# pritishnahar95/nvidia-terraform-modules

Hardware: AMD Instinct MI355X
Metric: cluster time-to-GPU-ready (s) + validation HIP GEMM TFLOPS at 1/2/4/8 MI355X (higher is better)
Workload: dtype bf16

## Files before the change

### nvidia_terraform_modules_amd/ops/_lib.py

```python
from __future__ import annotations

import ctypes
import os
from pathlib import Path

import torch

_HERE = Path(__file__).resolve().parent
LIB_PATH = _HERE / "libntm_validation.so"
EXP_LIB_PATH = _HERE / "libntm_experimental.so"

_lib: ctypes.CDLL | None = None
_exp: ctypes.CDLL | None = None


class NativeLibraryMissing(RuntimeError):
    pass


c_int, c_size, c_float, c_vp = ctypes.c_int, ctypes.c_size_t, ctypes.c_float, ctypes.c_void_p
c_uint, c_u64, c_double = ctypes.c_uint, ctypes.c_ulonglong, ctypes.c_double
_c_vpp = ctypes.POINTER(c_vp)

SIGNATURES = {
# ... 94 lines not shown
    "ntm_cu_sweep_launch": ([c_vp, c_vp, c_uint, c_int, c_size, c_uint,
                             c_uint, c_int, c_vp], c_int),
    "ntm_cu_sweep_decode": ([c_uint, c_uint, c_vp], None),
    "ntm_cu_sweep_summarize": ([c_vp, c_size, c_uint, c_uint, c_int, c_vp, c_size],
                               c_size),
    "ntm_xcd_sweep_record_bytes": ([], c_int),
    "ntm_xcd_sweep_heads_bytes": ([], c_int),
    "ntm_xcd_sweep_tile_bytes": ([], c_int),
    "ntm_xcd_sweep_mfma_per_batch": ([], c_int),
    "ntm_xcd_sweep_gated": ([c_int, c_int], c_int),
    "ntm_xcd_sweep_read_launch": ([c_vp, c_size, c_uint, c_uint, c_uint, c_int,
                                   c_u64, c_uint, c_int, c_uint, c_vp, c_vp,
                                   c_vp], c_int),
    "ntm_xcd_sweep_mfma_launch": ([c_uint, c_uint, c_uint, c_uint,
                                   c_uint, c_int, c_uint, c_vp, c_vp, c_vp], c_int),
    "ntm_xcd_sweep_summarize": ([c_vp, c_size, c_int, c_int, c_uint, c_uint,
                                 c_u64, c_double, c_int, c_vp, c_size], c_size),
    "ntm_atomics_ops": ([], c_int),
    "ntm_atomics_op_name": ([c_int], ctypes.c_char_p),
    "ntm_atomics_slot_bytes": ([c_int], c_int),
    "ntm_atomics_record_bytes": ([], c_int),
    "ntm_atomics_exact": ([c_int, c_u64, c_u64], c_int),
    "ntm_atomics_rmw_shape_ok": ([c_int, c_u64, c_uint, c_uint, c_u64], c_int),
    "ntm_atomics_expected": ([c_int, c_u64, c_u64, c_u64, c_u64, c_vp], c_int),
    "ntm_atomics_rmw_launch": ([c_int, c_vp, c_u64, c_uint, c_uint, c_u64, c_u64, c_vp], c_int),
    "ntm_atomics_rmw_reference_launch": ([c_int, c_vp, c_u64, c_uint, c_uint, c_u64, c_u64, c_vp], c_int),
    "ntm_atomics_ticket_claim_bytes": ([c_uint, c_uint, c_uint], c_size),
    "ntm_atomics_counter_bytes": ([c_uint], c_size),
    "ntm_atomics_ticket_launch": ([c_vp, c_vp, c_uint, c_uint, c_uint, c_uint, c_vp], c_int),
    "ntm_atomics_handoff_slab_bytes": ([c_uint, c_uint], c_size),
    "ntm_atomics_handoff_init": ([c_vp, c_uint, c_uint, c_u64, c_uint, c_vp], c_int),
    "ntm_atomics_handoff_launch": ([c_vp, c_vp, c_vp, c_uint, c_uint, c_u64, c_uint, c_uint, c_vp], c_int),
    "ntm_atomics_summarize_rmw": ([c_int, c_vp, c_vp, c_u64, c_int, c_vp, c_size], c_size),
    "ntm_atomics_summarize_tickets": ([c_vp, c_vp, c_uint, c_uint, c_uint, c_int, c_vp, c_size], c_size),
    "ntm_atomics_summarize_handoff": ([c_vp, c_size, c_uint, c_uint, c_uint, c_uint, c_int, c_vp, c_size], c_size),
}

XGMI_SIGNATURES = {
    "ntm_xgmi_allreduce_bf16": ([_c_vpp, _c_vpp, _c_vpp, c_int, c_int, c_int, c_int, c_size,
                                 c_uint, c_vp, c_int, c_vp], c_int),
    "ntm_xgmi_allreduce_bf16_ex": ([_c_vpp, _c_vpp, _c_vpp, c_int, c_int, c_int, c_int, c_size,
                                    c_uint, c_vp, c_int, c_uint, c_uint, c_vp], c_int),
    "ntm_xgmi_signal_bytes": ([c_int], c_size),
    "ntm_malloc": ([_c_vpp, c_size, c_int], c_int),
    "ntm_free": ([c_vp], c_int),
    "ntm_memset_async": ([c_vp, c_int, c_size, c_vp], c_int),
    "ntm_ipc_handle": ([c_vp, c_vp], c_int),
    "ntm_ipc_open": ([c_vp, _c_vpp], c_int),
    "ntm_ipc_close": ([c_vp], c_int),
}


def declare(lib: ctypes.CDLL, signatures: dict) -> None:
    for name, (argt, rest) in signatures.items():
        fn = getattr(lib, name)
        fn.argtypes = argt
        fn.restype = rest


def _declare(lib: ctypes.CDLL) -> None:
    declare(lib, SIGNATURES)


def lib() -> ctypes.CDLL:
    global _lib
    if _lib is not None:
        return _lib
    if not LIB_PATH.exists():
        raise NativeLibraryMissing(
            f"{LIB_PATH} not found. Build it with "
            "`python -m nvidia_terraform_modules_amd.ops.build` (needs hipcc, gfx950)."
        )
    mode = os.RTLD_NOW | getattr(os, "RTLD_GLOBAL", 0)
    _lib = ctypes.CDLL(str(LIB_PATH), mode=mode)
    _declare(_lib)
    return _lib


def _declare_experimental(lib: ctypes.CDLL) -> None:
    gemm = [c_int, c_vp, c_vp, c_vp, c_int, c_int, c_int, c_int, c_int, c_int, c_vp]
    sig = {
        "ntm_experimental_version": ([], ctypes.c_char_p),
        "ntm_gemm_bf16_experimental": (gemm, c_int),
        "ntm_gemm_bf16_knob": (gemm, c_int),
        "ntm_gemm_bf16_ws_knob": ([c_int] + gemm, c_int),
        "ntm_gemm_bf16_stamp": (
            [c_int, c_vp, c_vp, c_vp, c_int, c_int, c_int, c_int, c_int, c_int, c_vp, c_vp], c_int),
        "ntm_mfma_f8_probe": ([c_vp, c_vp, c_vp, c_vp], c_int),
        "ntm_mx_mfma_probe": ([c_int, c_vp, c_vp, c_vp, c_vp, c_vp, c_vp], c_int),
        "ntm_mfma_rate": ([c_int, c_int, c_int, c_vp, c_vp, c_vp], c_int),
        "ntm_mfma_toggle": ([c_int, c_int, c_int, c_vp, c_vp, c_vp], c_int),
        "ntm_dma_probe": ([c_int, c_vp, c_int, c_int, c_int, c_int, c_vp], c_int),
        "ntm_gemm_fp8_knob": ([c_vp, c_vp, c_vp, c_int, c_int, c_int, c_int, c_int, c_int, c_int,
                               c_vp], c_int),
        "ntm_gemm_bf16_sk_rev": ([c_vp, c_vp, c_vp, c_int, c_int, c_int, c_int, c_int, c_int,
                                  c_vp, c_size, c_vp], c_int),
        "ntm_gemm_bf16_sk_nopair": ([c_vp, c_vp, c_vp, c_int, c_int, c_int, c_int, c_int, c_int,
                                     c_vp, c_size, c_vp], c_int),
        "ntm_gemm_bf16_sk_stamp": ([c_vp, c_vp, c_vp, c_int, c_int, c_int, c_int, c_int, c_int,
                                    c_vp, c_size, c_vp, c_vp], c_int),
        "ntm_gemm_bf16_pp6_stamp": ([c_int, c_int, c_vp, c_vp, c_vp, c_int, c_int, c_int, c_int,
                                     c_int, c_int, c_vp, c_vp], c_int),
    }
    declare(lib, sig)


def lib_experimental() -> ctypes.CDLL:
    global _exp
    if _exp is not None:
        return _exp
    lib()
    if not EXP_LIB_PATH.exists():
        raise NativeLibraryMissing(
            f"{EXP_LIB_PATH} not found. Build it with "
            "`python -m nvidia_terraform_modules_amd.ops.build`.")
    _exp = ctypes.CDLL(str(EXP_LIB_PATH), mode=os.RTLD_NOW | getattr(os, "RTLD_GLOBAL", 0))
    _declare_experimental(_exp)
    return _exp


def available() -> bool:
    try:
        lib()
        return True
    except (NativeLibraryMissing, OSError):
        return False


def check(rc: int, what: str) -> None:
    if rc != 0:
        raise RuntimeError(f"{what} failed with hipError {rc}")


def stream_handle(stream: "torch.cuda.Stream | None" = None) -> int:
    if stream is None:
        stream = torch.cuda.current_stream()
    return int(stream.cuda_stream)


def version() -> str:
    return lib().ntm_version().decode()
```

### nvidia_terraform_modules_amd/ops/kernels.py

```python
from __future__ import annotations

import ctypes
from dataclasses import dataclass

import torch

from ._lib import check, lib, lib_experimental, stream_handle
from .mx import MX_BLOCK, mx_bits, mx_format_id, mx_shape_ok

BM = BN = 256
BK = 64


def gemm_shape_ok(m: int, n: int, k: int) -> bool:
    return m > 0 and n > 0 and k >= 2 * BK and m % BM == 0 and n % BN == 0 and k % BK == 0


def _require(t: torch.Tensor, name: str, dtype: torch.dtype) -> None:
    if not t.is_cuda:
        raise ValueError(f"{name} must be a GPU tensor")
    if t.dtype != dtype:
        raise ValueError(f"{name} must be {dtype}, got {t.dtype}")
    if t.dim() != 2 or t.stride(1) != 1:
        raise ValueError(f"{name} must be 2-D with unit inner stride")


GEMM_VARIANTS = {"default": 0, "pingpong8": 1, "pingpong8b": 4,
                 "pingpong8c": 5, "pingpong8cw": 10, "pingpong8cwe": 11,
                 "pingpong8cwn": 12, "pingpong8cwne": 13, "tile128": 15,
                 "tile256x128": 16, "tile160": 17, "tile256x160": 18, "tile128w4": 19,
                 "tile256x128w4": 20, "tile160w4": 21, "pingpong8cm": 22, "tile160x128": 23,
                 "tile128x160": 24, "tile128x256": 26, "pingpong8o": 25,
                 "pp8o_g128": 41, "pp8o_g128_nostore": 42, "pp8o_nostore": 43,
                 "pingpong8om": 47, "pingpong8od": 48, "pingpong8s": 49,
                 "pingpong8omd": 51, "pp192x256": 27, "pp256x192": 28,
                 "pp224x256": 29, "pp192x256s": 54, "pp256x192s": 55,
                 "dma4k_d3": 39}


EXPERIMENTAL_VARIANTS = frozenset({"pingpong8", "pingpong8cw",
                                   "pingpong8cwe", "pingpong8cwn", "pingpong8cwne",
                                   "tile128w4", "tile256x128w4", "tile160w4",
                                   "pp8o_g128", "pp8o_g128_nostore", "pp8o_nostore",
                                   "pingpong8od", "pingpong8omd", "pingpong8om", "pp224x256"})

TILE_SHAPES = {"tile128": (128, 128), "tile256x128": (256, 128), "tile160": (160, 160),
               "tile256x160": (256, 160), "tile128w4": (128, 128), "tile256x128w4": (256, 128),
               "tile160w4": (160, 160), "tile160x128": (160, 128), "tile128x160": (128, 160),
               "tile128x256": (128, 256)}


MASKED_TILES = frozenset({"tile128", "tile256x128", "tile160", "tile160x128", "tile128x160",
                          "tile128x256"})


def _tile128_shape_ok(m: int, n: int, k: int, tm: int = 128, tn: int = 128,
                      masked: bool = False) -> bool:
    if masked:
        return m > 0 and n > 0 and n % 4 == 0 and k > 0 and k % 8 == 0
    return m > 0 and n > 0 and m % tm == 0 and n % tn == 0 and k >= 128 and k % 128 == 0


def k1_plan(m: int, n: int, k: int) -> tuple[int, str, str]:
    top, tv, rest = ctypes.c_int(), ctypes.c_int(), ctypes.c_int()
    rc = lib().ntm_k1_plan(m, n, k, ctypes.byref(top), ctypes.byref(tv), ctypes.byref(rest))
    if rc != 0:
        raise ValueError(f"shape ({m},{n},{k}) not tiled by the K1 kernels")
    names = {v: kname for kname, v in GEMM_VARIANTS.items()}
    return top.value, names[tv.value], names[rest.value]


def k1_splitk_plan(m: int, n: int, k: int) -> tuple[int, str, str, int]:
    top, tv, rest, sp = ctypes.c_int(), ctypes.c_int(), ctypes.c_int(), ctypes.c_int()
    rc = lib().ntm_k1_plan_splitk(m, n, k, ctypes.byref(top), ctypes.byref(tv),
                                  ctypes.byref(rest), ctypes.byref(sp))
    if rc != 0:
        raise ValueError(f"shape ({m},{n},{k}) not tiled by the K1 kernels")
    names = {v: kname for kname, v in GEMM_VARIANTS.items()}
    return top.value, names[tv.value], names[rest.value], sp.value


_DEFAULT_WS: dict[tuple[int, int, int], int] = {}


_DEFAULT_SK: dict[tuple[int, int, int], str] = {}

SKH_VARIANTS = ("pp192x256s", "pp256x192s")
SK_VARIANTS = ("pingpong8s",) + SKH_VARIANTS


def k1_candidates(m: int, n: int, k: int, lda: int | None = None, ldb: int | None = None,
                  ldc: int | None = None) -> list[str]:
    lda, ldb, ldc = lda or k, ldb or k, ldc or n
    ok = (m % 256 == 0 and n % 256 == 0 and k % 128 == 0 and k >= 256 and
          not (lda % 8 or ldb % 8 or ldc % 8) and m * lda * 2 < (1 << 31) and
          n * ldb * 2 < (1 << 31))
    return ["default", "dma4k_d3"] if ok else ["default"]


def set_plan_pp_tiles(on: bool = True, split: bool | None = None) -> None:
    split = on if split is None else split
    lib().ntm_set_plan_pp_tiles((1 if on else 0) | (2 if split else 0))
    _DEFAULT_WS.clear()
    _DEFAULT_SK.clear()
    _FP8_WS.clear()


def set_plan_splitk(margin: float = 0.0, long_slice_k: int = -1, fp8: bool = True) -> None:
    lib().ntm_set_plan_splitk(float(margin), int(long_slice_k), 1 if fp8 else 0)
    _DEFAULT_WS.clear()
    _DEFAULT_SK.clear()
    _FP8_WS.clear()


def set_plan_splitk_ragged(on: bool = True) -> None:
    lib().ntm_set_plan_splitk_ragged(1 if on else 0)
    _DEFAULT_WS.clear()
    _DEFAULT_SK.clear()
    _FP8_WS.clear()


def set_cus_override(cus: int = 0) -> None:
    lib().ntm_set_cus_override(int(cus))
    _DEFAULT_WS.clear()
    _DEFAULT_SK.clear()
    _FP8_WS.clear()


def skh_ws_bytes(variant: str, m: int, n: int, k: int) -> int:
    if m <= 0 or n <= 0 or k <= 0:
        return 0
    return int(lib().ntm_skh_ws_bytes(GEMM_VARIANTS[variant], m, n, k))


def _default_ws_bytes(m: int, n: int, k: int) -> int:
    key = (m, n, k)
    wsb = _DEFAULT_WS.get(key)
    if wsb is None:
        _, top, _, sp = k1_splitk_plan(m, n, k)
        if top in SK_VARIANTS:
            ok = (sk_ws_bytes(m, n, k) if top == "pingpong8s" else skh_ws_bytes(top, m, n, k)) > 0
            wsb = -1 if ok else 0
            if ok:
                _DEFAULT_SK[key] = top
        else:
            wsb = lib().ntm_splitk_ws_bytes(m, n, k, sp) if sp > 1 else 0
        _DEFAULT_WS[key] = wsb
    return wsb


def gemm_bf16(a: torch.Tensor, b: torch.Tensor, out: torch.Tensor | None = None,
              variant: str = "default", splits: int = 1) -> torch.Tensor:
    _require(a, "a", torch.bfloat16)
    _require(b, "b", torch.bfloat16)
    m, k = a.shape
    n, kb = b.shape
    if k != kb:
        raise ValueError(f"K mismatch: a has {k}, b has {kb}")
    if variant in TILE_SHAPES:
        tm, tn = TILE_SHAPES[variant]
        if not _tile128_shape_ok(m, n, k, tm, tn, masked=variant in MASKED_TILES):
            raise ValueError(f"shape ({m},{n},{k}) not served by the {tm}x{tn} kernel "
                             "(masked tiles: N % 4, K % 8; others: whole tiles, K % 128)")
    elif variant == "default":
        _default_ws_bytes(m, n, k)
    elif variant in SKH_VARIANTS:
        if not skh_ws_bytes(variant, m, n, k):
            raise ValueError(f"shape ({m},{n},{k}) not served by {variant} (N % 8, K % 8, "
                             "K >= 128; at most half a round of its tiles, >= 2 K slices each)")
    elif variant in ("pingpong8s", "pingpong8s_rev", "pingpong8s_nopair"):
        if not sk_ws_bytes(m, n, k):
            raise ValueError(f"shape ({m},{n},{k}) not served by stream-K (N % 8, K % 8, K >= 128; "
                             "256x256 tiles: more than the CUs and not a multiple of them, or "
                             "few enough for >= 2 K slices per tile in one round)")
    elif variant in ("pingpong8cm", "pingpong8om", "pingpong8omd", "pp192x256", "pp256x192",
                     "pp224x256"):
        if not (m > 0 and n > 0 and n % 8 == 0 and k > 0 and k % 8 == 0):
            raise ValueError(f"shape ({m},{n},{k}) not served by {variant} (N % 8, K % 8)")
    elif not gemm_shape_ok(m, n, k):
        raise ValueError(f"shape ({m},{n},{k}) not tiled by the 256x256x64 kernel")
    if out is None:
        out = torch.empty((m, n), dtype=torch.bfloat16, device=a.device)
    _require(out, "out", torch.bfloat16)
    if tuple(out.shape) != (m, n):
        raise ValueError("out has the wrong shape")
    if variant in ("pingpong8s", "pingpong8s_rev", "pingpong8s_nopair"):
        return _gemm_bf16_sk(a, b, out, rev=variant == "pingpong8s_rev",
                             nopair=variant == "pingpong8s_nopair")
    if variant in SKH_VARIANTS:
        return _gemm_bf16_sk(a, b, out, sk_variant=variant)
    if splits > 1:
        if variant not in MASKED_TILES:
            raise ValueError(f"split-K runs on {sorted(MASKED_TILES)}, not {variant}")
        ws_bytes = lib().ntm_splitk_ws_bytes(m, n, k, splits)
        ws = torch.empty((ws_bytes + 3) // 4, dtype=torch.float32, device=a.device)
        rc = lib().ntm_gemm_bf16_splitk(
            GEMM_VARIANTS[variant], splits, a.data_ptr(), b.data_ptr(), out.data_ptr(), m, n, k,
            a.stride(0), b.stride(0), out.stride(0), ws.data_ptr(), ws_bytes, stream_handle())
        check(rc, "ntm_gemm_bf16_splitk")
        return out
    if variant.startswith("knob"):
        rc = lib_experimental().ntm_gemm_bf16_knob(
            int(variant[4:]), a.data_ptr(), b.data_ptr(), out.data_ptr(), m, n, k, a.stride(0),
            b.stride(0), out.stride(0), stream_handle())
        check(rc, "ntm_gemm_bf16_knob")
        return out
    if variant in EXPERIMENTAL_VARIANTS:
        rc = lib_experimental().ntm_gemm_bf16_experimental(
            GEMM_VARIANTS[variant], a.data_ptr(), b.data_ptr(), out.data_ptr(), m, n, k,
            a.stride(0), b.stride(0), out.stride(0), stream_handle())
        check(rc, "ntm_gemm_bf16_experimental")
        return out
    if variant == "default" and _default_ws_bytes(m, n, k) < 0:
        return _gemm_bf16_sk(a, b, out, sk_variant=_DEFAULT_SK[(m, n, k)])
    if variant == "default" and _default_ws_bytes(m, n, k):
        wsb = _default_ws_bytes(m, n, k)
        ws = torch.empty((wsb + 3) // 4, dtype=torch.float32, device=a.device)
        rc = lib().ntm_gemm_bf16_ex(a.data_ptr(), b.data_ptr(), out.data_ptr(), m, n, k,
                                    a.stride(0), b.stride(0), out.stride(0), ws.data_ptr(), wsb,
                                    stream_handle())
        check(rc, "ntm_gemm_bf16_ex")
        return out
    rc = lib().ntm_gemm_bf16_variant(
        GEMM_VARIANTS[variant], a.data_ptr(), b.data_ptr(), out.data_ptr(), m, n, k,
        a.stride(0), b.stride(0), out.stride(0), stream_handle())
    check(rc, "ntm_gemm_bf16")
    return out


def sk_ws_bytes(m: int, n: int, k: int) -> int:
    if m <= 0 or n <= 0 or k <= 0:
        return 0
    return int(lib().ntm_sk_ws_bytes(m, n, k))


_SK_WS: dict[tuple[int, int], torch.Tensor] = {}


def _sk_workspace(dev: torch.device, nbytes: int) -> torch.Tensor:
    key = (dev.index if dev.index is not None else torch.cuda.current_device(),
           int(stream_handle() or 0))
    ws = _SK_WS.get(key)
    if ws is None or ws.numel() * 4 < nbytes:
        ws = torch.zeros((nbytes + 3) // 4, dtype=torch.float32, device=dev)
        _SK_WS[key] = ws
    return ws


def sk_xcc_error(device=None, clear: bool = True) -> int:
    dev = torch.device(device) if device is not None else torch.device(
        "cuda", torch.cuda.current_device())
    key = (dev.index if dev.index is not None else torch.cuda.current_device(),
           int(stream_handle() or 0))
    ws = _SK_WS.get(key)
    if ws is None:
        return 0
    i = lib().ntm_sk_error_word_index()
    word = ws.view(torch.int32)[i:i + 1]
    v = int(word.item()) & 0xFFFFFFFF
    if clear and v:
        word.zero_()
# ... 1034 lines not shown
```

### validation/src/ntm_experimental.hip

```cpp
#include "ntm/dma_probe.hpp"
#include "ntm/gemm_bf16.hpp"
#include "ntm/gemm_bf16_pp3.hpp"
#include "ntm/gemm_bf16_pp3h.hpp"
#include "ntm/gemm_bf16_pp3_stamp.hpp"
#include "ntm/gemm_bf16_pp6.hpp"
#include "ntm/gemm_bf16_sk.hpp"
#include "ntm/gemm_w4k.hpp"
#include "ntm/gemm_bf16_t128.hpp"
#include "ntm/gemm_fp8_diag.hpp"
#include "ntm/mx_gemm.hpp"
#include "ntm/stream_policy_exp.hpp"

#include "ntm/abi.h"

namespace {
inline hipStream_t S(void* s) { return reinterpret_cast<hipStream_t>(s); }
using ntm::gemm::make_args;
}

NTM_API const char* ntm_experimental_version() { return "ntm-experimental 0.2.0 gfx950"; }

NTM_API int ntm_gemm_bf16_experimental(int variant, const void* A, const void* B, void* C, int M,
                                       int N, int K, int lda, int ldb, int ldc, void* stream) {
  const ntm::gemm::GemmArgs a = make_args(A, B, C, M, N, K, lda, ldb, ldc);
  switch (variant) {
    case 1: return (int)ntm::gemm::launch_gemm_bf16(a, S(stream));
    case 10:
    case 11:
    case 12:
    case 13: return (int)ntm::gemm3::launch_gemm_bf16_pp3_knob(a, variant + 2, S(stream));
    case 39: return (int)ntm::w4k::launch_gemm_bf16_w4k<3>(a, S(stream));
    case 19: return (int)ntm::gemmt::launch_gemm_bf16_tile<4>(a, S(stream));
    case 20: return (int)ntm::gemmt::launch_gemm_bf16_tile<8>(a, S(stream));
    case 21: return (int)ntm::gemmt::launch_gemm_bf16_tile<5, 5>(a, S(stream));
    case 41: return (int)ntm::gemm6::launch_gemm_bf16_pp6_grid<1>(a, 128, S(stream));
    case 42: return (int)ntm::gemm6::launch_gemm_bf16_pp6_grid<2>(a, 128, S(stream));
    case 43: return (int)ntm::gemm6::launch_gemm_bf16_pp6_grid<2>(a, 256, S(stream));
    case 48: return (int)ntm::gemm6::launch_gemm_bf16_pp6<1, 0, true>(a, S(stream));
    case 47:
      if (!ntm::gemm6::shape_ok6m(M, N, K) || (lda % 8) || (ldb % 8) || (ldc % 8))
        return (int)ntm::gemm3::launch_gemm_bf16_pp3_masked(a, S(stream));
      return (int)ntm::gemm6::launch_gemm_bf16_pp6_masked<1>(a, S(stream));
    case 29: return (int)ntm::gemm3h::launch_gemm_bf16_pp3h<96, 128>(a, S(stream));
    case 51: return (int)ntm::gemm6::launch_gemm_bf16_pp6_masked<1, true>(a, S(stream));
    default: return (int)hipErrorInvalidValue;
  }
}

NTM_API int ntm_gemm_bf16_sk_rev(const void* A, const void* B, void* C, int M, int N, int K,
                                 int lda, int ldb, int ldc, void* ws, size_t ws_bytes,
                                 void* stream) {
  const ntm::gemm::GemmArgs a = make_args(A, B, C, M, N, K, lda, ldb, ldc);
  return (int)ntm::gemmsk::launch_gemm_bf16_sk<true>(a, ntm::gemm6::pp6_grid(1 << 30), ws,
                                                     ws_bytes, S(stream));
}

NTM_API int ntm_gemm_bf16_sk_stamp(const void* A, const void* B, void* C, int M, int N, int K,
                                   int lda, int ldb, int ldc, void* ws, size_t ws_bytes,
                                   void* stamps, void* stream) {
  const ntm::gemm::GemmArgs a = make_args(A, B, C, M, N, K, lda, ldb, ldc);
  return (int)ntm::gemmsk::launch_gemm_bf16_sk<false, true>(
      a, ntm::gemm6::pp6_grid(1 << 30), ws, ws_bytes, S(stream), (unsigned long long*)stamps);
}

NTM_API int ntm_gemm_bf16_sk_nopair(const void* A, const void* B, void* C, int M, int N, int K,
                                    int lda, int ldb, int ldc, void* ws, size_t ws_bytes,
                                    void* stream) {
  const ntm::gemm::GemmArgs a = make_args(A, B, C, M, N, K, lda, ldb, ldc);
  return (int)ntm::gemmsk::launch_gemm_bf16_sk<false, false, false>(
      a, ntm::gemm6::pp6_grid(1 << 30), ws, ws_bytes, S(stream));
}

NTM_API int ntm_gemm_bf16_pp6_oddcut(int cut_pairs, const void* A, const void* B, void* C, int M,
                                     int N, int K, int lda, int ldb, int ldc, void* stream) {
  ntm::gemm::GemmArgs a = make_args(A, B, C, M, N, K, lda, ldb, ldc);
  a.splitk_kc = cut_pairs;
  return (int)ntm::gemm6::launch_gemm_bf16_pp6<1, 3, true>(a, S(stream));
}

NTM_API int ntm_gemm_bf16_pp6_stamp(int grid, int store, const void* A, const void* B, void* C,
                                    int M, int N, int K, int lda, int ldb, int ldc, void* stamps,
                                    void* stream) {
  ntm::gemm::GemmArgs a = make_args(A, B, C, M, N, K, lda, ldb, ldc);
  a.stamps = (unsigned long long*)stamps;
  if (grid * 2 > (M / 256) * (N / 256)) return (int)hipErrorInvalidValue;
  using namespace ntm::gemm6;
  switch (store) {
    case 0: return (int)launch_gemm_bf16_pp6_grid<2, 2>(a, grid, S(stream));
    case 1: return (int)launch_gemm_bf16_pp6_grid<1, 2>(a, grid, S(stream));
    case 2: return (int)launch_gemm_bf16_pp6_grid<1, 2, true>(a, grid, S(stream));
    default: return (int)hipErrorInvalidValue;
  }
}

NTM_API int ntm_gemm_bf16_knob(int knob, const void* A, const void* B, void* C, int M, int N,
                               int K, int lda, int ldb, int ldc, void* stream) {
  return (int)ntm::gemm3::launch_gemm_bf16_pp3_knob(make_args(A, B, C, M, N, K, lda, ldb, ldc),
                                                    knob, S(stream));
}

NTM_API int ntm_gemm_bf16_stamp(int mode, const void* A, const void* B, void* C, int M, int N,
                                int K, int lda, int ldb, int ldc, void* stamps, void* stream) {
  return (int)ntm::gemm3s::launch_gemm_bf16_pp3_stamp(make_args(A, B, C, M, N, K, lda, ldb, ldc),
                                                      mode, (unsigned long long*)stamps, S(stream));
}

NTM_API int ntm_mfma_rate(int f8, int grid, int iters, void* out, float* sink, void* stream) {
  if (grid <= 0 || iters <= 0) return (int)hipErrorInvalidValue;
  if (f8 == 3)
    hipLaunchKernelGGL((ntm::fp8::mfma_rate_kernel<true, true>), dim3(grid), dim3(256), 0,
                       S(stream), iters, 7u, (unsigned long long*)out, sink);
  else if (f8 == 2)
    hipLaunchKernelGGL((ntm::fp8::mfma_rate_kernel<false, true>), dim3(grid), dim3(256), 0,
                       S(stream), iters, 7u, (unsigned long long*)out, sink);
  else if (f8)
    hipLaunchKernelGGL(ntm::fp8::mfma_rate_kernel<true>, dim3(grid), dim3(256), 0, S(stream),
                       iters, 7u, (unsigned long long*)out, sink);
  else
    hipLaunchKernelGGL(ntm::fp8::mfma_rate_kernel<false>, dim3(grid), dim3(256), 0, S(stream),
                       iters, 7u, (unsigned long long*)out, sink);
  return (int)hipGetLastError();
}

NTM_API int ntm_mfma_toggle(int pat, int grid, int iters, void* out, float* sink, void* stream) {
  if (grid <= 0 || iters <= 0) return (int)hipErrorInvalidValue;
  auto* o = (unsigned long long*)out;
  switch (pat) {
#define NTM_TOGGLE(P)                                                                         \
  case P:                                                                                     \
// ... 104 lines not shown
```

### validation/src/ntm_validation.hip

```cpp
#include "ntm/atomics.hpp"
#include "ntm/aux_kernels.hpp"
#include "ntm/cu_sweep.hpp"
#include "ntm/gemm_bf16_pp2.hpp"
#include "ntm/gemm_bf16_pp3.hpp"
#include "ntm/gemm_bf16_pp3h.hpp"
#include "ntm/gemm_bf16_pp6.hpp"
#include "ntm/gemm_bf16_sk.hpp"
#include "ntm/gemm_bf16_skh.hpp"
#include "ntm/gemm_bf16_t128.hpp"
#include "ntm/gemm_fp8.hpp"
#include "ntm/gemm_w4k.hpp"
#include "ntm/hbm_pattern.hpp"
#include "ntm/host_link.hpp"
#include "ntm/mx_gemm.hpp"
#include "ntm/xcd_sweep.hpp"

#include "ntm/abi.h"

namespace {
inline hipStream_t S(void* s) { return reinterpret_cast<hipStream_t>(s); }
inline unsigned stream_grid(size_t work_items, unsigned block) {
  size_t g = (work_items + block - 1) / block;
  if (g > 2048) g = 2048;
  if (g == 0) g = 1;
  return (unsigned)g;
}
}

NTM_API const char* ntm_version() { return "ntm-validation 0.1.0 gfx950"; }

NTM_API int ntm_gemm_shape_ok(int M, int N, int K) {
  return ntm::gemm::shape_ok(M, N, K) ? 1 : 0;
}

namespace k1 = ntm::k1;

constexpr bool kPp6Spread = true;

static k1::PlanKnobs g_knobs;
NTM_API void ntm_set_plan_pp_tiles(int on) {
  g_knobs.pp = (on & 1) != 0;
  g_knobs.pp_split = (on & 2) != 0;
}
NTM_API void ntm_set_plan_splitk(double margin, int long_k, int fp8_long) {
  g_knobs.splitk_margin = margin > 0.0 ? margin : 0.0;
  g_knobs.splitk_min_k = long_k >= 0 ? long_k : -1;
  g_knobs.splitk_fp8_long = fp8_long != 0;
}
NTM_API void ntm_set_plan_splitk_ragged(int on) { g_knobs.splitk_ragged = on != 0; }

inline k1::PlanQuery query(int M, int N, int K, bool splitk, bool fp8) {
  return k1::PlanQuery{M, N, K, ntm::gemm6::device_cus(), splitk, fp8, g_knobs};
}
inline k1::K1Plan plan_k1(int M, int N, int K, bool splitk = false, bool fp8 = false) {
  return k1::plan(query(M, N, K, splitk, fp8));
}
inline int put_plan(const k1::K1Plan& pl, int* top_rows, int* top_variant, int* rest_variant,
                    int* splits = nullptr) {
  if (!pl.feasible()) return (int)hipErrorInvalidValue;
  *top_rows = pl.top_rows;
  *top_variant = pl.top_variant;
  *rest_variant = pl.rest_variant;
  if (splits) *splits = pl.splits;
  return 0;
}

NTM_API int ntm_pp3h_vmcnt(int ah, int bh, int phase) {
  using namespace ntm::gemm3h;
  if (phase < 0 || phase > 3) return -1;
  int v[4];
  auto fill = [&](auto geo) {
    using G = decltype(geo);
    v[0] = G::vmc(0), v[1] = G::vmc(1), v[2] = G::vmc(2), v[3] = G::vmc(3);
  };
  if (ah == 64 && bh == 128) fill(Geo<64, 128>{});
  else if (ah == 128 && bh == 64) fill(Geo<128, 64>{});
  else if (ah == 96 && bh == 128) fill(Geo<96, 128>{});
  else if (ah == 128 && bh == 128) fill(Geo<128, 128>{});
  else return -1;
  return v[phase];
}

NTM_API int ntm_k1_plan_times(int M, int N, int K, double* unsplit_s, double* sk_s) {
  if (!unsplit_s || !sk_s) return (int)hipErrorInvalidValue;
  const k1::K1Plan pl = plan_k1(M, N, K, true);
  if (!pl.feasible()) return (int)hipErrorInvalidValue;
  *unsplit_s = pl.unsplit_s;
  *sk_s = pl.sk_s;
  return 0;
}

NTM_API int ntm_k1_plan(int M, int N, int K, int* top_rows, int* top_variant, int* rest_variant) {
  if (M <= 0 || N <= 0 || K <= 0 || !top_rows || !top_variant || !rest_variant)
    return (int)hipErrorInvalidValue;
  return put_plan(plan_k1(M, N, K), top_rows, top_variant, rest_variant);
}

NTM_API int ntm_k1_plan_splitk(int M, int N, int K, int* top_rows, int* top_variant,
                               int* rest_variant, int* splits) {
  if (M <= 0 || N <= 0 || K <= 0 || !top_rows || !top_variant || !rest_variant || !splits)
    return (int)hipErrorInvalidValue;
  return put_plan(plan_k1(M, N, K, true), top_rows, top_variant, rest_variant, splits);
}

template <int I = 0, typename F>
inline int with_ws_tile(int variant, F&& f) {
  if constexpr (I < k1::kNumSmallTiles) {
    constexpr k1::SmallTile st = k1::kSmallTiles[I];
    if constexpr (st.masked && !st.pp) {
      if (variant == st.variant)
        return (int)f(std::integral_constant<int, st.tm / 32>{},
                      std::integral_constant<int, st.tn / 32>{});
    }
    return with_ws_tile<I + 1>(variant, f);
  }
  return (int)hipErrorInvalidValue;
}
static_assert(k1::small_tile(k1::kTile256x160).tm == ntm::gemmt::Cfg<8, 5>::TM &&
              k1::small_tile(k1::kTile256x160).tn == ntm::gemmt::Cfg<8, 5>::TN);
static_assert(k1::small_tile(k1::kPp192x256).tm == ntm::gemm3h::Geo<64, 128>::TM &&
              k1::small_tile(k1::kPp192x256).tn == ntm::gemm3h::Geo<64, 128>::TN);
static_assert(k1::small_tile(k1::kPp256x192).tm == ntm::gemm3h::Geo<128, 64>::TM &&
              k1::small_tile(k1::kPp256x192).tn == ntm::gemm3h::Geo<128, 64>::TN);

NTM_API int ntm_gemm_bf16_variant(int variant, const void* A, const void* B,
                                  void* C, int M, int N, int K, int lda,
                                  int ldb, int ldc, void* stream) {
  if (variant == k1::kPlan) {
    const k1::K1Plan pl = plan_k1(M, N, K);
    if (!pl.feasible()) return (int)hipErrorInvalidValue;
    if (pl.top_rows < M) {
      const int rc = ntm_gemm_bf16_variant(pl.top_variant, A, B, C, pl.top_rows, N, K, lda, ldb,
                                           ldc, stream);
      if (rc != 0) return rc;
      return ntm_gemm_bf16_variant(pl.rest_variant, (const __bf16*)A + (size_t)pl.top_rows * lda,
                                   B, (__bf16*)C + (size_t)pl.top_rows * ldc, M - pl.top_rows, N,
                                   K, lda, ldb, ldc, stream);
    }
    variant = pl.top_variant;
  }
  const ntm::gemm::GemmArgs a = ntm::gemm::make_args(A, B, C, M, N, K, lda, ldb, ldc);
  switch (variant) {
    case k1::kPingpong8b: return (int)ntm::gemm2::launch_gemm_bf16_pp2(a, S(stream));
    case k1::kPingpong8c: return (int)ntm::gemm3::launch_gemm_bf16_pp3(a, S(stream));
    case k1::kPingpong8o:
      if (!ntm::gemm6::shape_ok6(M, N, K) || (lda % 8) || (ldb % 8) || (ldc % 8))
        return (int)ntm::gemm3::launch_gemm_bf16_pp3(a, S(stream));
      return (int)ntm::gemm6::launch_gemm_bf16_pp6<1, 0, kPp6Spread>(a, S(stream));
    case k1::kTile256x160: return (int)ntm::gemmt::launch_gemm_bf16_tile<8, 5>(a, S(stream));
    case k1::kPingpong8cm: return (int)ntm::gemm3::launch_gemm_bf16_pp3_masked(a, S(stream));
    case k1::kPp192x256: return (int)ntm::gemm3h::launch_gemm_bf16_pp3h<64, 128>(a, S(stream));
    case k1::kPp256x192: return (int)ntm::gemm3h::launch_gemm_bf16_pp3h<128, 64>(a, S(stream));
    case k1::kDma4kD3: return (int)ntm::w4k::launch_gemm_bf16_w4k<3>(a, S(stream));
    default:
      return with_ws_tile(variant, [&](auto mt, auto nt) {
        return ntm::gemmt::launch_gemm_bf16_tile_ws<decltype(mt)::value, decltype(nt)::value>(
            a, S(stream));
      });
  }
}

NTM_API size_t ntm_splitk_ws_bytes(int M, int N, int K, int splits) {
  if (M <= 0 || N <= 0 || K <= 0 || splits < 1) return 0;
  return sizeof(float) * (size_t)ntm::gemmt::splitk_slices(K, splits) * M * N;
}

NTM_API int ntm_gemm_bf16_splitk(int variant, int splits, const void* A, const void* B, void* C,
                                 int M, int N, int K, int lda, int ldb, int ldc, void* ws,
                                 size_t ws_bytes, void* stream) {
  if (splits < 1 || !ws || ws_bytes < ntm_splitk_ws_bytes(M, N, K, splits))
    return (int)hipErrorInvalidValue;
  const ntm::gemm::GemmArgs a = ntm::gemm::make_args(A, B, C, M, N, K, lda, ldb, ldc);
  return with_ws_tile(variant, [&](auto mt, auto nt) {
    return ntm::gemmt::launch_gemm_bf16_tile_ws_splitk<decltype(mt)::value, decltype(nt)::value>(
        a, splits, (float*)ws, S(stream));
  });
}

NTM_API int ntm_sk_error_word_index() { return ntm::gemmsk::kErrWord; }
NTM_API void ntm_set_sk_fault_inject(int v) { ntm::gemmsk::sk_fault_inject() = (unsigned)v; }

NTM_API int ntm_plan_cus() { return ntm::gemm6::device_cus(); }
NTM_API void ntm_set_cus_override(int cus) { ntm::gemm6::cu_override() = cus > 0 ? cus : 0; }

NTM_API size_t ntm_sk_ws_bytes(int M, int N, int K) {
  ntm::gemmsk::SkArgs s;
  if (!ntm::gemmsk::shape_ok_sk(M, N, K) ||
      !ntm::gemmsk::sk_decompose(M, N, K, ntm::gemm6::pp6_grid(1 << 30), s))
    return 0;
  return ntm::gemmsk::sk_ws_bytes(s.G);
}

NTM_API int ntm_gemm_bf16_sk(const void* A, const void* B, void* C, int M, int N, int K, int lda,
                             int ldb, int ldc, void* ws, size_t ws_bytes, void* stream) {
  const ntm::gemm::GemmArgs a = ntm::gemm::make_args(A, B, C, M, N, K, lda, ldb, ldc);
  return (int)ntm::gemmsk::launch_gemm_bf16_sk(a, ntm::gemm6::pp6_grid(1 << 30), ws, ws_bytes,
                                               S(stream));
}

NTM_API size_t ntm_skh_ws_bytes(int variant, int M, int N, int K) {
  ntm::gemmsk::SkArgs s;
  const int cus = ntm::gemm6::pp6_grid(1 << 30);
  if (!ntm::gemmsk::shape_ok_sk(M, N, K)) return 0;
  const bool ok = variant == k1::kPp192x256s   ? ntm::gemmskh::sk_decompose_h<192, 256>(M, N, K, cus, s)
                  : variant == k1::kPp256x192s ? ntm::gemmskh::sk_decompose_h<256, 192>(M, N, K, cus, s)
                                               : false;
  return ok ? ntm::gemmsk::sk_ws_bytes(s.G) : 0;
}

NTM_API int ntm_gemm_bf16_skh_ex(int variant, const void* A, const void* B, void* C, int M, int N,
                                 int K, int lda, int ldb, int ldc, void* ws, size_t ws_bytes,
                                 int fault, void* stream) {
  const ntm::gemm::GemmArgs a = ntm::gemm::make_args(A, B, C, M, N, K, lda, ldb, ldc);
  const int cus = ntm::gemm6::pp6_grid(1 << 30);
  if (variant == k1::kPp192x256s)
    return (int)ntm::gemmskh::launch_gemm_bf16_skh<64, 128>(a, cus, ws, ws_bytes, S(stream), fault);
  if (variant == k1::kPp256x192s)
    return (int)ntm::gemmskh::launch_gemm_bf16_skh<128, 64>(a, cus, ws, ws_bytes, S(stream), fault);
  return (int)hipErrorInvalidValue;
}

NTM_API int ntm_gemm_bf16_skh(int variant, const void* A, const void* B, void* C, int M, int N,
                              int K, int lda, int ldb, int ldc, void* ws, size_t ws_bytes,
                              void* stream) {
  return ntm_gemm_bf16_skh_ex(variant, A, B, C, M, N, K, lda, ldb, ldc, ws, ws_bytes, -1, stream);
}

NTM_API int ntm_gemm_bf16_ex(const void* A, const void* B, void* C, int M, int N, int K, int lda,
                             int ldb, int ldc, void* ws, size_t ws_bytes, void* stream) {
  if (ws) {
    const k1::K1Plan pl = plan_k1(M, N, K, true);
    if (pl.feasible() && pl.splits > 1 && ws_bytes >= ntm_splitk_ws_bytes(M, N, K, pl.splits))
      return ntm_gemm_bf16_splitk(pl.top_variant, pl.splits, A, B, C, M, N, K, lda, ldb, ldc, ws,
                                  ws_bytes, stream);
    if (pl.feasible() && pl.sk && pl.top_variant == k1::kPingpong8s &&
        ws_bytes >= ntm_sk_ws_bytes(M, N, K) &&
// ... 717 lines not shown
```

Baseline: 1611.

## Add five-slot LDS ring pipeline for the DMA 4K bf16 GEMM kernel

Adds a new w4r GEMM kernel that stages A/B tiles through a five-slot LDS ring filled by buffer-load-to-LDS. Each step interleaves the async loads for tile t+2 and the LDS fragment reads for the next step between the MFMA instructions, with a single barrier per K step and peeled remainder handling for T mod 5. The existing dma4k_d3 variant now routes to this kernel whenever its shape check passes, aiming to hide global-load latency better than the three-deep w4k pipeline. The deeper ring uses more LDS, and the hand-placed waitcnt and schedule barriers need to be correct for the results to be right.

```diff
diff --git a/nvidia_terraform_modules_amd/ops/_lib.py b/nvidia_terraform_modules_amd/ops/_lib.py
--- a/nvidia_terraform_modules_amd/ops/_lib.py
+++ b/nvidia_terraform_modules_amd/ops/_lib.py
@@ -200,6 +200,7 @@
     sig = {
         "ntm_experimental_version": ([], ctypes.c_char_p),
         "ntm_gemm_bf16_experimental": (gemm, c_int),
+        "ntm_w4r_shape_ok": ([c_int] * 6, c_int),
         "ntm_gemm_bf16_knob": (gemm, c_int),
         "ntm_gemm_bf16_ws_knob": ([c_int] + gemm, c_int),
         "ntm_gemm_bf16_stamp": (
diff --git a/nvidia_terraform_modules_amd/ops/kernels.py b/nvidia_terraform_modules_amd/ops/kernels.py
--- a/nvidia_terraform_modules_amd/ops/kernels.py
+++ b/nvidia_terraform_modules_amd/ops/kernels.py
@@ -35,14 +35,15 @@
                  "pingpong8om": 47, "pingpong8od": 48, "pingpong8s": 49,
                  "pingpong8omd": 51, "pp192x256": 27, "pp256x192": 28,
                  "pp224x256": 29, "pp192x256s": 54, "pp256x192s": 55,
-                 "dma4k_d3": 39}
+                 "dma4k_d3": 39, "dma4k_r5": 62}
 
 
 EXPERIMENTAL_VARIANTS = frozenset({"pingpong8", "pingpong8cw",
                                    "pingpong8cwe", "pingpong8cwn", "pingpong8cwne",
                                    "tile128w4", "tile256x128w4", "tile160w4",
                                    "pp8o_g128", "pp8o_g128_nostore", "pp8o_nostore",
-                                   "pingpong8od", "pingpong8omd", "pingpong8om", "pp224x256"})
+                                   "pingpong8od", "pingpong8omd", "pingpong8om", "pp224x256",
+                                   "dma4k_r5"})
 
 TILE_SHAPES = {"tile128": (128, 128), "tile256x128": (256, 128), "tile160": (160, 160),
                "tile256x160": (256, 160), "tile128w4": (128, 128), "tile256x128w4": (256, 128),
@@ -96,6 +97,14 @@
           not (lda % 8 or ldb % 8 or ldc % 8) and m * lda * 2 < (1 << 31) and
           n * ldb * 2 < (1 << 31))
     return ["default", "dma4k_d3"] if ok else ["default"]
+
+
+def w4r_shape_ok(m: int, n: int, k: int, lda: int | None = None, ldb: int | None = None,
+                 ldc: int | None = None) -> bool:
+    lda, ldb, ldc = lda or k, ldb or k, ldc or n
+    return (m > 0 and n > 0 and m % 256 == 0 and n % 256 == 0 and k % 128 == 0 and k >= 384 and
+            lda >= k and ldb >= k and ldc >= n and not (lda % 8 or ldb % 8 or ldc % 8) and
+            m * lda * 2 < (1 << 31) and n * ldb * 2 < (1 << 31))
 
 
 def set_plan_pp_tiles(on: bool = True, split: bool | None = None) -> None:
@@ -177,6 +186,10 @@
                      "pp224x256"):
         if not (m > 0 and n > 0 and n % 8 == 0 and k > 0 and k % 8 == 0):
             raise ValueError(f"shape ({m},{n},{k}) not served by {variant} (N % 8, K % 8)")
+    elif variant == "dma4k_r5":
+        if not w4r_shape_ok(m, n, k, a.stride(0), b.stride(0), None if out is None else out.stride(0)):
+            raise ValueError(f"shape ({m},{n},{k}) not served by {variant} (M, N % 256, K % 128, "
+                             "K >= 384, rows 16-byte aligned, operands < 2 GiB)")
     elif not gemm_shape_ok(m, n, k):
         raise ValueError(f"shape ({m},{n},{k}) not tiled by the 256x256x64 kernel")
     if out is None:
diff --git a/validation/include/ntm/gemm_w4r.hpp b/validation/include/ntm/gemm_w4r.hpp
--- /dev/null
+++ b/validation/include/ntm/gemm_w4r.hpp
@@ -0,0 +1,179 @@
+#pragma once
+
+#include "ntm/gemm_w4k.hpp"
+
+namespace ntm {
+namespace w4r {
+
+using ::ntm::gemm::GemmArgs;
+using ::ntm::gemm::raw_barrier;
+using ::ntm::w4k::Ctx;
+using ::ntm::w4k::Frags8;
+using ::ntm::w4k::kOp;
+
+constexpr int kSlots = 5;
+constexpr int kLds = kSlots * kOp;
+static_assert(kLds >= ::ntm::w4k::kLds, "the C staging aliases the ring");
+constexpr int kMinTiles = 6;
+constexpr int kNA0 = 4, kDI = 4;
+
+__device__ __forceinline__ void ring_piece(const Ctx& c, int kt, int T, int slot, int w, int i) {
+  const int kb = (kt < T ? kt : T - 1) * 128;
+  const bool is_b = i >= 8;
+  const int rbi = (i >> 1) & 3, ks = i & 1;
+  char* dst = c.lds + slot * kOp + ((w * 4 + rbi) * 2 + ks) * 1024;
+  __builtin_amdgcn_raw_ptr_buffer_load_lds(is_b ? c.rsb : c.rsa, (NTM_AS3 void*)dst, 16,
+                                           is_b ? c.voff_b : c.voff_a,
+                                           kb + ks * 64 + rbi * (is_b ? c.rowblk_b : c.rowblk_a),
+                                           0, 0);
+}
+
+struct Bases {
+  int a[3], b[3];
+};
+
+__device__ __forceinline__ void ring_bases(const Ctx& c, Bases& r) {
+#pragma unroll
+  for (int h = 0; h < 3; ++h) {
+    r.a[h] = c.rd_a + h * 2 * kOp;
+    r.b[h] = c.rd_b - kOp + h * 2 * kOp;
+    asm volatile("" : "+v"(r.a[h]), "+v"(r.b[h]));
+  }
+}
+
+__device__ __forceinline__ void ring_read_a(const Ctx& c, const Bases& r, Frags8& f, int slot,
+                                            int mt) {
+  const char* p = c.lds + r.a[slot >> 1] + ((slot & 1) * kOp + mt * 2048);
+  f.a[mt][0] = *(const bf16x8*)p;
+  f.a[mt][1] = *(const bf16x8*)(p + 1024);
+}
+
+__device__ __forceinline__ void ring_read_b(const Ctx& c, const Bases& r, Frags8& f, int slot,
+                                            int nt) {
+  const char* p = c.lds + r.b[slot >> 1] + ((slot & 1) * kOp + nt * 2048);
+  f.b[nt][0] = *(const bf16x8*)p;
+  f.b[nt][1] = *(const bf16x8*)(p + 1024);
+}
+
+template <int U, int NA0, int DI>
+__device__ __forceinline__ void step(const Ctx& c, const Bases& r, f32x4 (&acc)[8][8], Frags8& f, int t, int T,
+                                     int w) {
+  static_assert(NA0 == 0 || NA0 == 2 || NA0 == 4 || NA0 == 8, "A(t+2) pieces in row 0");
+  static_assert(DI >= 1 && (15 - NA0) * DI <= 55, "the other pieces within rows 1..7");
+  constexpr int sA1 = (2 * U + 2) % kSlots, sB1 = (2 * U + 3) % kSlots;
+  constexpr int sA2 = (2 * U + 4) % kSlots, sB2 = (2 * U) % kSlots;
+#pragma unroll
+  for (int nt = 0; nt < 8; ++nt) {
+    ::ntm::w4k::mma<false>(acc[0][nt], f, 0, nt);
+    if constexpr (NA0 > 0)
+      if (nt % (8 / NA0) == 0) ring_piece(c, t + 2, T, sA2, w, nt / (8 / NA0));
+    __builtin_amdgcn_sched_barrier(0);
+  }
+  asm volatile("s_waitcnt vmcnt(%0)" ::"n"(NA0) : "memory");
+  asm volatile("s_waitcnt lgkmcnt(0)" ::: "memory");
+  raw_barrier();
+#pragma unroll
+  for (int mt = 1; mt < 8; ++mt) {
+#pragma unroll
+    for (int nt = 0; nt < 8; ++nt) {
+      ::ntm::w4k::mma<false>(acc[mt][nt], f, mt, nt);
+      const int j = (mt - 1) * 8 + nt;
+      if ((j % DI) == 0 && j / DI < 16 - NA0) {
+        const int i = NA0 + j / DI;
+        ring_piece(c, t + 2, T, i < 8 ? sA2 : sB2, w, i);
+      }
+      if (nt == 1) ring_read_a(c, r, f, sA1, mt - 1);
+      if (mt == 7) ring_read_b(c, r, f, sB1, nt);
+      __builtin_amdgcn_sched_barrier(0);
+    }
+  }
+  ring_read_a(c, r, f, sA1, 7);
+  __builtin_amdgcn_sched_barrier(0);
+}
+
+__device__ __forceinline__ void ring_prologue(const Ctx& c, const Bases& r, Frags8& f, int T, int w) {
+#pragma unroll
+  for (int i = 0; i < 16; ++i) ring_piece(c, 0, T, i < 8 ? 0 : 1, w, i);
+#pragma unroll
+  for (int i = 0; i < 16; ++i) ring_piece(c, 1, T, i < 8 ? 2 : 3, w, i);
+  asm volatile("s_waitcnt vmcnt(16)" ::: "memory");
+  raw_barrier();
+#pragma unroll
+  for (int i = 0; i < 8; ++i) {
+    ring_read_a(c, r, f, 0, i);
+    ring_read_b(c, r, f, 1, i);
+  }
+}
+
+template <int NA0, int DI>
+__device__ __forceinline__ void group(const Ctx& c, const Bases& r, f32x4 (&acc)[8][8], Frags8& f, int t, int T,
+                                      int w) {
+  step<0, NA0, DI>(c, r, acc, f, t, T, w);
+  step<1, NA0, DI>(c, r, acc, f, t + 1, T, w);
+  step<2, NA0, DI>(c, r, acc, f, t + 2, T, w);
+  step<3, NA0, DI>(c, r, acc, f, t + 3, T, w);
+  step<4, NA0, DI>(c, r, acc, f, t + 4, T, w);
+}
+
+template <int NA0, int DI, int R>
+__global__ void __launch_bounds__(::ntm::w4k::kThreads, 1) gemm_w4r_kernel(GemmArgs p) {
+  static_assert(R >= 0 && R < kSlots, "T % 5");
+  __shared__ __attribute__((aligned(16))) char smem[kLds];
+  Ctx c;
+  int m0, n0, lane, w, wr, wc;
+  ::ntm::w4k::setup(p, smem, c, m0, n0, lane, w, wr, wc);
+  f32x4 acc[8][8];
+#pragma unroll
+  for (int i = 0; i < 8; ++i)
+#pragma unroll
+    for (int j = 0; j < 8; ++j) acc[i][j] = f32x4{0.f, 0.f, 0.f, 0.f};
+
+  const int T = p.K / 64;
+  Frags8 f;
+  Bases r;
+  ring_bases(c, r);
+  ring_prologue(c, r, f, T, w);
+  const int t_peel = T - (R ? R : kSlots);
+  int t = 0;
+  do {
+    group<NA0, DI>(c, r, acc, f, t, T, w);
+    t += kSlots;
+  } while (t < t_peel);
+  if constexpr (R == 0) {
+    group<NA0, DI>(c, r, acc, f, t, T, w);
+  } else {
+    step<0, NA0, DI>(c, r, acc, f, t, T, w);
+    if constexpr (R > 1) step<1, NA0, DI>(c, r, acc, f, t + 1, T, w);
+    if constexpr (R > 2) step<2, NA0, DI>(c, r, acc, f, t + 2, T, w);
+    if constexpr (R > 3) step<3, NA0, DI>(c, r, acc, f, t + 3, T, w);
+  }
+
+  ::ntm::gemm::mfma_drain();
+  asm volatile("s_waitcnt vmcnt(0)" ::: "memory");
+  asm volatile("s_waitcnt lgkmcnt(0)" ::: "memory");
+  raw_barrier();
+  ::ntm::w4k::store_tile<true>(p, smem, acc, m0, n0, w, wr, wc, lane);
+}
+
+inline bool shape_ok(int M, int N, int K, int lda, int ldb, int ldc) {
+  return M > 0 && N > 0 && K >= kMinTiles * 64 && !(M % ::ntm::w4k::BM) && !(N % ::ntm::w4k::BN) &&
+         !(K % 128) && lda >= K && ldb >= K && ldc >= N && !(lda % 8) && !(ldb % 8) && !(ldc % 8) &&
+         (long long)M * lda * 2 < (1ll << 31) && (long long)N * ldb * 2 < (1ll << 31);
+}
+
+template <int NA0 = kNA0, int DI = kDI>
+inline hipError_t launch_gemm_bf16_w4r(const GemmArgs& a, hipStream_t stream) {
+  if (!shape_ok(a.M, a.N, a.K, a.lda, a.ldb, a.ldc) || a.rowsum) return hipErrorInvalidValue;
+  const dim3 g((unsigned)((a.M / ::ntm::w4k::BM) * (a.N / ::ntm::w4k::BN))), b(::ntm::w4k::kThreads);
+  switch ((a.K / 64) % kSlots) {
+    case 0: hipLaunchKernelGGL((gemm_w4r_kernel<NA0, DI, 0>), g, b, 0, stream, a); break;
+    case 1: hipLaunchKernelGGL((gemm_w4r_kernel<NA0, DI, 1>), g, b, 0, stream, a); break;
+    case 2: hipLaunchKernelGGL((gemm_w4r_kernel<NA0, DI, 2>), g, b, 0, stream, a); break;
+    case 3: hipLaunchKernelGGL((gemm_w4r_kernel<NA0, DI, 3>), g, b, 0, stream, a); break;
+    default: hipLaunchKernelGGL((gemm_w4r_kernel<NA0, DI, 4>), g, b, 0, stream, a); break;
+  }
+  return hipGetLastError();
+}
+
+}
+}
diff --git a/validation/src/ntm_experimental.hip b/validation/src/ntm_experimental.hip
--- a/validation/src/ntm_experimental.hip
+++ b/validation/src/ntm_experimental.hip
@@ -6,6 +6,7 @@
 #include "ntm/gemm_bf16_pp6.hpp"
 #include "ntm/gemm_bf16_sk.hpp"
 #include "ntm/gemm_w4k.hpp"
+#include "ntm/gemm_w4r.hpp"
 #include "ntm/gemm_bf16_t128.hpp"
 #include "ntm/gemm_fp8_diag.hpp"
 #include "ntm/mx_gemm.hpp"
@@ -30,6 +31,7 @@
     case 12:
     case 13: return (int)ntm::gemm3::launch_gemm_bf16_pp3_knob(a, variant + 2, S(stream));
     case 39: return (int)ntm::w4k::launch_gemm_bf16_w4k<3>(a, S(stream));
+    case 62: return (int)ntm::w4r::launch_gemm_bf16_w4r<>(a, S(stream));
     case 19: return (int)ntm::gemmt::launch_gemm_bf16_tile<4>(a, S(stream));
     case 20: return (int)ntm::gemmt::launch_gemm_bf16_tile<8>(a, S(stream));
     case 21: return (int)ntm::gemmt::launch_gemm_bf16_tile<5, 5>(a, S(stream));
@@ -45,6 +47,10 @@
     case 51: return (int)ntm::gemm6::launch_gemm_bf16_pp6_masked<1, true>(a, S(stream));
     default: return (int)hipErrorInvalidValue;
   }
+}
+
+NTM_API int ntm_w4r_shape_ok(int M, int N, int K, int lda, int ldb, int ldc) {
+  return ntm::w4r::shape_ok(M, N, K, lda, ldb, ldc) ? 1 : 0;
 }
 
 NTM_API int ntm_gemm_bf16_sk_rev(const void* A, const void* B, void* C, int M, int N, int K,
diff --git a/validation/src/ntm_validation.hip b/validation/src/ntm_validation.hip
--- a/validation/src/ntm_validation.hip
+++ b/validation/src/ntm_validation.hip
@@ -10,6 +10,7 @@
 #include "ntm/gemm_bf16_t128.hpp"
 #include "ntm/gemm_fp8.hpp"
 #include "ntm/gemm_w4k.hpp"
+#include "ntm/gemm_w4r.hpp"
 #include "ntm/hbm_pattern.hpp"
 #include "ntm/host_link.hpp"
 #include "ntm/mx_gemm.hpp"
@@ -151,7 +152,9 @@
     case k1::kPingpong8cm: return (int)ntm::gemm3::launch_gemm_bf16_pp3_masked(a, S(stream));
     case k1::kPp192x256: return (int)ntm::gemm3h::launch_gemm_bf16_pp3h<64, 128>(a, S(stream));
     case k1::kPp256x192: return (int)ntm::gemm3h::launch_gemm_bf16_pp3h<128, 64>(a, S(stream));
-    case k1::kDma4kD3: return (int)ntm::w4k::launch_gemm_bf16_w4k<3>(a, S(stream));
+    case k1::kDma4kD3:
+      if (ntm::w4r::shape_ok(M, N, K, lda, ldb, ldc)) return (int)ntm::w4r::launch_gemm_bf16_w4r<>(a, S(stream));
+      return (int)ntm::w4k::launch_gemm_bf16_w4k<3>(a, S(stream));
     default:
       return with_ws_tile(variant, [&](auto mt, auto nt) {
         return ntm::gemmt::launch_gemm_bf16_tile_ws<decltype(mt)::value, decltype(nt)::value>(
```

New measurement: 1611 (median of 3 runs). Within noise of the previous version (+0.0%).
